# mkkellogg/GaussianSplats3D

Hardware: NVIDIA H100
Metric: frames_per_sec (higher is better)
Workload: dtype int32 sort keys / f32 raster

## Files before the change

gaussiansplats3d_b200/csrc/common.cuh:

```cuda
#pragma once
#include <cuda_runtime.h>
#include <stdint.h>
#include <stdio.h>
#include "../../include/gsplat_b200.h"

extern thread_local char g_gs_err[512];

#include <vector>
#include <string.h>
#include <stdlib.h>

namespace gs {

template <typename T, bool PINNED> struct GpuBuf {
    T *p = nullptr;
    size_t n = 0;
    GpuBuf() = default;
    GpuBuf(const GpuBuf &) = delete;
    GpuBuf &operator=(const GpuBuf &) = delete;
    ~GpuBuf() { release(); }
    int ensure(size_t count) {
        if (count <= n) return GS_OK;
        release();
        const size_t bytes = (count ? count : 1) * sizeof(T);
// ... 109 lines not shown
__device__ __forceinline__ uint32_t block_exclusive_scan(uint32_t v, uint32_t *smem_warp , uint32_t &total) {
    const int lane = threadIdx.x & 31, warp = threadIdx.x >> 5;
    constexpr int NW = THREADS / 32;
    const uint32_t inc = warp_inclusive_scan(v);
    if (lane == 31) smem_warp[warp] = inc;
    __syncthreads();
    if (warp == 0) {
        uint32_t w = lane < NW ? smem_warp[lane] : 0u;
        uint32_t wi = warp_inclusive_scan(w);
        smem_warp[lane] = wi - w;
        if (lane == 31) smem_warp[32] = wi;
    }
    __syncthreads();
    const uint32_t r = inc - v + smem_warp[warp];
    total = smem_warp[32];
    __syncthreads();
    return r;
}

struct SortControl {
    int32_t dmin, dmax;
    uint32_t error;
    uint32_t hist[4][kRadix];
};
constexpr uint32_t kErrDegenerate = 1u;
constexpr uint32_t kErrBucketRange = 2u;
constexpr uint32_t kErrCapacity = 4u;

}
```

gaussiansplats3d_b200/csrc/engine.cu:

```cuda
#include "../../include/gsplat_b200.h"
#include "common.cuh"
#include "sort_kernels.cuh"
#include "raster_kernels.cuh"
#include "shard_kernels.cuh"
#include "ksplat_transform.h"
#include "ksplat_kernels.cuh"
#include "file_kernels.cuh"
#include "cull_kernels.cuh"
#include "ray_kernels.cuh"
#include "generate_kernels.cuh"

#include <algorithm>
#include <cmath>
#include <cstdarg>
#include <cstdlib>
#include <cstring>
#include <memory>
#include <new>
#include <vector>

using namespace gs;

thread_local char g_gs_err[512] = "";
#define g_err g_gs_err
// ... 141 lines not shown
        if (graph_exec) cudaGraphExecDestroy(graph_exec);
        if (graph_exec_alt) cudaGraphExecDestroy(graph_exec_alt);
        for (cudaEvent_t x : ev) if (x) cudaEventDestroy(x);
        for (int i = 0; i < kPipeRing; ++i) { if (ev_frame_done[i]) cudaEventDestroy(ev_frame_done[i]); if (ev_copy_done[i]) cudaEventDestroy(ev_copy_done[i]); }
        for (cudaEvent_t x : {ev_params[0], ev_params[1], ev_fork, ev_join}) if (x) cudaEventDestroy(x);
        for (cudaStream_t x : {stream, stream2, copy_stream, param_stream}) if (x) cudaStreamDestroy(x);
    }
};

static int check_engine(gs_engine *e) {
    if (!e) return fail(GS_ERR_BAD_ARG, "null engine");
    cudaError_t ce = cudaSetDevice(e->cfg.device);
    if (ce != cudaSuccess) return fail(GS_ERR_CUDA, "cudaSetDevice(%d) -> %s", e->cfg.device, cudaGetErrorString(ce));
    return GS_OK;
}

extern "C" int gs_create(const gs_config *cfg, gs_engine **out) {
    if (!cfg || !out) return fail(GS_ERR_BAD_ARG, "gs_create: null argument");
    *out = nullptr;
    gs_config c{};
    memcpy(&c, cfg, std::min<size_t>(cfg->struct_size ? cfg->struct_size : sizeof(gs_config), sizeof(gs_config)));
    if (c.distance_map_range == 0) c.distance_map_range = 1u << 16;
    if (c.distance_map_range < 2 || c.distance_map_range > (1u << 24)) return fail(GS_ERR_BAD_ARG, "distance_map_range %u outside [2, 2^24]", c.distance_map_range);
    if (c.world_size == 0) { c.world_size = 1; c.rank = 0; }
    if (c.rank >= c.world_size) return fail(GS_ERR_BAD_ARG, "rank %u >= world_size %u", c.rank, c.world_size);
    int ndev = gs_device_count();
    if (ndev <= 0) return fail(GS_ERR_NO_DEVICE, "no CUDA device visible: libgsplat_b200 has no CPU path");
    if (c.device < 0 || c.device >= ndev) return fail(GS_ERR_BAD_ARG, "device %d not in [0,%d)", c.device, ndev);
    CU(cudaSetDevice(c.device));
    std::unique_ptr<gs_engine> e(new (std::nothrow) gs_engine());
    if (!e) return fail(GS_ERR_BAD_ARG, "out of host memory");
    e->cfg = c;
    cudaDeviceProp prop{};
    CU(cudaGetDeviceProperties(&prop, c.device));
    e->sm_count = prop.multiProcessorCount;
    if (prop.l2CacheSize > 0) e->l2_bytes = (size_t)prop.l2CacheSize;
    CU(cudaStreamCreateWithFlags(&e->stream, cudaStreamNonBlocking));
    CU(cudaStreamCreateWithFlags(&e->stream2, cudaStreamNonBlocking));
    CU(cudaEventCreateWithFlags(&e->ev_fork, cudaEventDisableTiming));
    CU(cudaEventCreateWithFlags(&e->ev_join, cudaEventDisableTiming));
    for (int i = 0; i < EV_COUNT; ++i) CU(cudaEventCreate(&e->ev[i]));
    int kb = 0;
    while ((1u << kb) < c.distance_map_range) ++kb;
    e->key_bits = kb;
    int rc = GS_OK;
    const size_t n = std::max<uint32_t>(c.max_splat_count, 1);
// ... 53 lines not shown
    P.irow[0] = (int32_t)((double)mvp[2] * 1000.0);
    P.irow[1] = (int32_t)((double)mvp[6] * 1000.0);
    P.irow[2] = (int32_t)((double)mvp[10] * 1000.0);
    P.irow[3] = 1;
    P.frow[0] = mvp[2]; P.frow[1] = mvp[6]; P.frow[2] = mvp[10]; P.frow[3] = 0.f;
    if (!capturing) CU(cudaMemcpyAsync(e->depthp.p + e->rs.frame_parity, &P, sizeof(P), cudaMemcpyHostToDevice, st));
    const bool integer = e->cfg.integer_based_sort, dyn = e->cfg.dynamic_mode;
    const int mode = use_pre ? (integer ? kIntPrecomputed : kFloatPrecomputed)
                             : (integer ? (dyn ? kIntDynamic : kIntStatic) : (dyn ? kFloatDynamic : kFloatStatic));
    const int dblocks = (int)std::max<uint64_t>(1, std::min<uint64_t>(((uint64_t)n + kDepthThreads * kDepthItems - 1) / (kDepthThreads * kDepthItems), (uint64_t)e->sm_count * 8));
    const bool identity = (d_indexes == nullptr);
    const void *pre = e->precomputed.p;
    switch (mode) {
        case kIntStatic: launch_depth<kIntStatic>(identity, dblocks, st, d_indexes, e->centers.p, pre, e->scene_idx.p, e->transforms.p, e->depthp.p + e->rs.frame_parity, lo, hi, e->dist.p, e->ctl.p); break;
        case kIntDynamic: launch_depth<kIntDynamic>(identity, dblocks, st, d_indexes, e->centers.p, pre, e->scene_idx.p, e->transforms.p, e->depthp.p + e->rs.frame_parity, lo, hi, e->dist.p, e->ctl.p); break;
        case kIntPrecomputed: launch_depth<kIntPrecomputed>(identity, dblocks, st, d_indexes, e->centers.p, pre, e->scene_idx.p, e->transforms.p, e->depthp.p + e->rs.frame_parity, lo, hi, e->dist.p, e->ctl.p); break;
        case kFloatStatic: launch_depth<kFloatStatic>(identity, dblocks, st, d_indexes, e->centers.p, pre, e->scene_idx.p, e->transforms.p, e->depthp.p + e->rs.frame_parity, lo, hi, e->dist.p, e->ctl.p); break;
        case kFloatDynamic: launch_depth<kFloatDynamic>(identity, dblocks, st, d_indexes, e->centers.p, pre, e->scene_idx.p, e->transforms.p, e->depthp.p + e->rs.frame_parity, lo, hi, e->dist.p, e->ctl.p); break;
        default: launch_depth<kFloatPrecomputed>(identity, dblocks, st, d_indexes, e->centers.p, pre, e->scene_idx.p, e->transforms.p, e->depthp.p + e->rs.frame_parity, lo, hi, e->dist.p, e->ctl.p); break;
    }
    return GS_OK;
}

static int sort_on_device(gs_engine *e, const uint32_t *d_indexes, const float *mvp, uint32_t sort_count, uint32_t render_count,
                          bool use_pre, bool write_buckets, bool capturing = false, bool subset = false, cudaEvent_t wait_for_rects = nullptr) {
    if (sort_count > render_count) return fail(GS_ERR_BAD_ARG, "sortCount %u > renderCount %u", sort_count, render_count);
    if (render_count > e->cfg.max_splat_count) return fail(GS_ERR_CAPACITY, "renderCount %u > max_splat_count %u", render_count, e->cfg.max_splat_count);
    cudaStream_t st = e->stream;
    const uint32_t s0 = render_count - sort_count, n = sort_count;
    const PassPlan pl = make_plan_bits(e->key_bits);
    uint32_t launches = 0;
    uint32_t stride = 0;
    int rc = e->tile_hist.ensure(radix_tile_hist_words(std::max(n, 1u), pl.npasses, &stride));
    if (rc) return rc;
    if (!capturing) CU(cudaEventRecord(e->ev[EV_SORT0], st));
    if (!e->have_prof_begin) e->prof.begin(st);
    if (e->ctl_dirty && !capturing) {
        gs_launch(k_sort_init, 1, 256, 0, st, e->ctl.p);
        ++launches;
    }
    if (!capturing) e->ctl_dirty = true;
    if (s0 > 0) { gs_launch(k_copy_head, std::min<uint32_t>((s0 + 255) / 256, e->sm_count * 8), 256, 0, st, d_indexes, e->sorted.p, s0); ++launches; e->prof.mark("k_copy_head", st); }
    if (n > 0) {
        if ((rc = enqueue_depth(e, d_indexes, mvp, use_pre, s0, render_count, capturing))) return rc;
        const bool identity = (d_indexes == nullptr);
        ++launches;
        e->prof.mark("k_depth", st);
        if (!capturing) CU(cudaEventRecord(e->ev[EV_DEPTH], st));
        const uint32_t tiles = (n + kRadixTile - 1) / kRadixTile;
        const uint32_t R = e->cfg.distance_map_range;
        const uint32_t *vsrc = identity ? nullptr : d_indexes + s0;
        int vmode = identity ? kValIotaReversed : kValArrayReversed;
        int32_t *dist_sorted = e->dist.p + s0;
        const unsigned long long *n_dev = nullptr;
        if (subset) {
            if (wait_for_rects) CU(cudaStreamWaitEvent(st, wait_for_rects, 0));
            int rcs = raster_subset(e->rs, e->cfg, d_indexes, render_count, e->dist.p, e->sub_idx.p, e->sub_dist.p, st, e->prof, launches);
            if (rcs) return rcs;
            vsrc = e->sub_idx.p; vmode = kValArrayReversed;
            dist_sorted = e->sub_dist.p;
            n_dev = &e->rs.rctl.p->subset_count;
        }
        static const RadixNames names = {{"k_radix_hist[depth,0]", "k_radix_hist[depth,1]", "k_radix_hist[depth,2]", "k_radix_hist[depth,3]"},
                                         {"k_radix_scan[depth,0]", "k_radix_scan[depth,1]", "k_radix_scan[depth,2]", "k_radix_scan[depth,3]"},
                                         {"k_radix_scatter[depth,0]", "k_radix_scatter[depth,1]", "k_radix_scatter[depth,2]", "k_radix_scatter[depth,3]"}};
        if (e->key_bits <= 16) {
            gs_launch(k_bucket<uint16_t>, tiles, kRadixThreads, 0, st, dist_sorted, (uint16_t *)e->keys[0].p, n, n_dev, R, pl, write_buckets ? 1 : 0, e->ctl.p, e->tile_hist.p, stride);
            ++launches;
            e->prof.mark("k_bucket", st);
            if (!capturing) CU(cudaEventRecord(e->ev[EV_BUCKET], st));
            radix_sort_pairs<uint16_t, uint32_t>((uint16_t *)e->keys[0].p, (uint16_t *)e->keys[1].p, vsrc, render_count - 1u, vmode, e->vals[0].p, e->vals[1].p,
                                       e->sorted.p + s0, n, n_dev, (unsigned long long)n, pl, e->ctl.p, e->tile_hist.p, stride, true, nullptr, st, launches, &e->prof, names, true);
        } else {
            gs_launch(k_bucket<uint32_t>, tiles, kRadixThreads, 0, st, dist_sorted, e->keys[0].p, n, n_dev, R, pl, write_buckets ? 1 : 0, e->ctl.p, e->tile_hist.p, stride);
            ++launches;
            e->prof.mark("k_bucket", st);
            if (!capturing) CU(cudaEventRecord(e->ev[EV_BUCKET], st));
            radix_sort_pairs<uint32_t, uint32_t>(e->keys[0].p, e->keys[1].p, vsrc, render_count - 1u, vmode, e->vals[0].p, e->vals[1].p, e->sorted.p + s0, n,
                                       n_dev, (unsigned long long)n, pl, e->ctl.p, e->tile_hist.p, stride, true, nullptr, st, launches, &e->prof, names, true);
        }
    } else if (!capturing) {
        CU(cudaEventRecord(e->ev[EV_DEPTH], st));
        CU(cudaEventRecord(e->ev[EV_BUCKET], st));
    }
    if (!capturing) CU(cudaEventRecord(e->ev[EV_SORT1], st));
    CU(cudaGetLastError());
    e->tm.kernel_launches = launches;
    e->last_render_count = render_count;
    e->have_sorted = true;
    if (!capturing) e->ctl_dirty = false;
    return GS_OK;
}

static int finish_sort(gs_engine *e, float *sort_time_ms) {
    CU(cudaMemcpyAsync(e->h_ctl.p, e->ctl.p, 12, cudaMemcpyDeviceToHost, e->stream));
    CU(cudaStreamSynchronize(e->stream));
    float ms = 0.f;
    if (e->last_frame_was_graph) {
        e->tm.depth_ms = e->tm.bucket_ms = e->tm.scatter_ms = 0.f;
        cudaEventElapsedTime(&ms, e->ev[EV_SORT0], e->ev[EV_R1]);
    } else {
        cudaEventElapsedTime(&e->tm.depth_ms, e->ev[EV_SORT0], e->ev[EV_DEPTH]);
        cudaEventElapsedTime(&e->tm.bucket_ms, e->ev[EV_DEPTH], e->ev[EV_BUCKET]);
// ... 47 lines not shown
    cudaEventElapsedTime(&e->tm.d2h_ms, e->ev[EV_D2H0], e->ev[EV_D2H1]);
    return rc;
}


static int shard_prepare(gs_engine *e) {
    const uint32_t R = e->cfg.distance_map_range;
    int rc;
    const size_t bytes = sizeof(ShardHeader) + (size_t)R * sizeof(uint2);
    if (e->shard.block.n < bytes) {
        if ((rc = e->shard.block.ensure(bytes))) return rc;
        CU(cudaMemset(e->shard.block.p, 0, bytes));
    }
    const size_t blocks = ((size_t)R + kShardScanThreads - 1) / kShardScanThreads;
    if ((rc = e->shard.total.ensure(R)) || (rc = e->shard.ahead.ensure(R)) || (rc = e->shard.delta.ensure(R)) || (rc = e->shard.block_total.ensure(blocks)) ||
        (rc = e->shard.local_sorted.ensure(e->cfg.max_splat_count)))
        return rc;
    const PassPlan pl = make_plan_bits(e->key_bits);
    if ((rc = e->tile_hist.ensure(radix_tile_hist_words(std::max(e->cfg.max_splat_count, 1u), pl.npasses, nullptr))) || (rc = e->precomputed.ensure(e->cfg.max_splat_count))) return rc;
    return GS_OK;
}
template <typename F> static inline void preload_kernel(F f) { cudaFuncAttributes a; (void)cudaFuncGetAttributes(&a, f); }
template <typename KeyT> static void shard_preload_keyed() {
    preload_kernel(k_bucket<KeyT>);
    preload_kernel(k_radix_hist<KeyT>);
    preload_kernel(k_shard_place<KeyT>);
    preload_kernel(k_radix_scatter<KeyT, uint32_t, kValArray, true, false>);
    preload_kernel(k_radix_scatter<KeyT, uint32_t, kValArrayReversed, true, false>);
    preload_kernel(k_radix_scatter<KeyT, uint32_t, kValIotaReversed, true, false>);
    preload_kernel(k_radix_scatter<KeyT, uint32_t, kValArray, true, true>);
    preload_kernel(k_radix_scatter<KeyT, uint32_t, kValArrayReversed, true, true>);
    preload_kernel(k_radix_scatter<KeyT, uint32_t, kValIotaReversed, true, true>);
}
template <int MODE> static void shard_preload_depth() { preload_kernel(k_depth<MODE, true>); preload_kernel(k_depth<MODE, false>); }
static void shard_preload(gs_engine *e) {
    preload_kernel(k_sort_init); preload_kernel(k_copy_head); preload_kernel(k_radix_scan);
    preload_kernel(k_shard_exchange_minmax); preload_kernel(k_shard_exchange_runs); preload_kernel(k_shard_totals); preload_kernel(k_shard_delta); preload_kernel(k_shard_done);
    shard_preload_depth<kIntStatic>(); shard_preload_depth<kIntDynamic>(); shard_preload_depth<kIntPrecomputed>();
    shard_preload_depth<kFloatStatic>(); shard_preload_depth<kFloatDynamic>(); shard_preload_depth<kFloatPrecomputed>();
    if (e->key_bits <= 16) shard_preload_keyed<uint16_t>(); else shard_preload_keyed<uint32_t>();
    (void)cudaGetLastError();
}
static inline ShardHeader *shard_hdr(void *block) { return (ShardHeader *)block; }
static inline const uint2 *shard_runs(void *block) { return (const uint2 *)((unsigned char *)block + sizeof(ShardHeader)); }

extern "C" int gs_shard_export(gs_engine *e, void *block_handle, void *sorted_handle) {
    int rc = check_engine(e);
// ... 62 lines not shown
        if ((rc = shard_prepare(pe))) return rc;
        blocks[g] = pe->shard.block.p;
    }
    return shard_bind(e, world, blocks, engines[0]->sorted.p);
}

template <typename KeyT>
static int shard_local_sort(gs_engine *e, const uint32_t *d_indexes, uint32_t s0, uint32_t lo, uint32_t hi, uint32_t &launches) {
    cudaStream_t st = e->stream;
    const uint32_t n = hi - lo, R = e->cfg.distance_map_range;
    const PassPlan pl = make_plan_bits(e->key_bits);
    uint32_t stride = 0;
    int rc = e->tile_hist.ensure(radix_tile_hist_words(std::max(n, 1u), pl.npasses, &stride));
    if (rc) return rc;
    const bool identity = (d_indexes == nullptr);
    static const RadixNames names = {{"k_radix_hist[shard,0]", "k_radix_hist[shard,1]", "k_radix_hist[shard,2]", "k_radix_hist[shard,3]"},
                                     {"k_radix_scan[shard,0]", "k_radix_scan[shard,1]", "k_radix_scan[shard,2]", "k_radix_scan[shard,3]"},
                                     {"k_radix_scatter[shard,0]", "k_radix_scatter[shard,1]", "k_radix_scatter[shard,2]", "k_radix_scatter[shard,3]"}};
    const uint32_t me = e->cfg.rank, world = e->shard.world, seq = e->shard.seq;
    uint2 *runs = (uint2 *)shard_runs(e->shard.block.p);
    KeyT *final_keys = nullptr;
    if (n) {
        const uint32_t tiles = (n + kRadixTile - 1) / kRadixTile;
        gs_launch(k_bucket<KeyT>, tiles, kRadixThreads, 0, st, e->dist.p + lo, (KeyT *)e->keys[0].p, n, nullptr, R, pl, 0, e->ctl.p, e->tile_hist.p, stride);
        ++launches;
        e->prof.mark("k_bucket", st);
        radix_sort_pairs<KeyT, uint32_t>((KeyT *)e->keys[0].p, (KeyT *)e->keys[1].p, identity ? nullptr : d_indexes + lo, hi - 1u,
                                         identity ? kValIotaReversed : kValArrayReversed, e->vals[0].p, e->vals[1].p, e->shard.local_sorted.p, n, nullptr,
                                         (unsigned long long)n, pl, e->ctl.p, e->tile_hist.p, stride, true, runs, st, launches, &e->prof, names, true, true, &final_keys);
    }
    k_shard_exchange_runs<<<1, 32, 0, st>>>(e->shard.peers, me, world, seq);
    ++launches;
    e->prof.mark("k_shard_exchange_runs", st);
    if (n) {
        const uint32_t sblocks = (R + kShardScanThreads - 1) / kShardScanThreads;
        k_shard_totals<<<sblocks, kShardScanThreads, 0, st>>>(e->shard.peers, me, world, R, e->shard.total.p, e->shard.ahead.p, e->shard.block_total.p);
        k_shard_delta<<<sblocks, kShardScanThreads, 0, st>>>(runs, R, e->shard.total.p, e->shard.ahead.p, e->shard.block_total.p, e->shard.delta.p);
        e->prof.mark("k_shard_offsets", st);
        k_shard_place<KeyT><<<std::min<uint32_t>((n + 255) / 256, e->sm_count * 16), 256, 0, st>>>(final_keys, e->shard.local_sorted.p, n, e->shard.delta.p, e->shard.root_out + s0);
        e->prof.mark("k_shard_place", st);
        launches += 3;
    }
    return GS_OK;
}

static inline uint32_t shard_bound(uint32_t s0, uint32_t n, uint32_t g, uint32_t world) { return s0 + (uint32_t)(((uint64_t)n * g) / world); }

// ... 1465 lines not shown
```

gaussiansplats3d_b200/csrc/sort_kernels.cuh:

```cuda
#pragma once
#include "common.cuh"

namespace gs {

enum DepthMode : int {
    kIntStatic = 0, kIntDynamic = 1, kIntPrecomputed = 2, kFloatStatic = 3, kFloatDynamic = 4, kFloatPrecomputed = 5
};

struct DepthParams {
    int32_t irow[4];
    float frow[4];
    float mvp[16];
};

__global__ void k_sort_init(SortControl *ctl) {
    pdl_enter();
    const uint32_t tid = threadIdx.x;
    if (tid == 0) {
        ctl->dmin = 2147483640;
        ctl->dmax = -2147483640;
        ctl->error = 0;
    }
    uint32_t *h = &ctl->hist[0][0];
    for (uint32_t i = tid; i < 4 * kRadix; i += blockDim.x) h[i] = 0;
// ... 51 lines not shown
    DepthParams P;
#pragma unroll
    for (int i = 0; i < 4; ++i) { P.irow[i] = __ldg(&Pp->irow[i]); P.frow[i] = __ldg(&Pp->frow[i]); }
    if (MODE == kIntDynamic || MODE == kFloatDynamic) {
#pragma unroll
        for (int i = 0; i < 16; ++i) P.mvp[i] = __ldg(&Pp->mvp[i]);
    }
    __shared__ int32_t s_irow[GS_MAX_SCENES_DEV][4];
    __shared__ float s_frow[GS_MAX_SCENES_DEV][4];
    __shared__ int s_min[kDepthThreads / 32], s_max[kDepthThreads / 32];
    if (MODE == kIntDynamic || MODE == kFloatDynamic) {
        if (threadIdx.x < GS_MAX_SCENES_DEV) {
            float row[4];
            scene_row(P.mvp, transforms + 16 * threadIdx.x, row);
#pragma unroll
            for (int k = 0; k < 4; ++k) {
                s_frow[threadIdx.x][k] = row[k];
                s_irow[threadIdx.x][k] = trunc_scaled(row[k], 1000.0);
            }
        }
        __syncthreads();
    }
    if (blockIdx.x == 0 && threadIdx.x == 0) ctl->error = 0;
    int32_t lmin = 2147483640, lmax = -2147483640;
    const uint32_t tile = kDepthThreads * kDepthItems;
    for (uint64_t base = (uint64_t)s0 + (uint64_t)blockIdx.x * tile; base < rc; base += (uint64_t)gridDim.x * tile) {
        uint32_t g[kDepthItems];
#pragma unroll
        for (int k = 0; k < kDepthItems; ++k) {
            const uint64_t i = base + (uint64_t)k * kDepthThreads + threadIdx.x;
            g[k] = (i < rc) ? (IDENTITY ? (uint32_t)i : ld_nc_u32(indexes + i)) : 0xffffffffu;
        }
        int32_t d[kDepthItems];
#pragma unroll
        for (int k = 0; k < kDepthItems; ++k)
            if (g[k] != 0xffffffffu) d[k] = splat_distance<MODE>(g[k], centers, pre, scene_idx, P, s_irow, s_frow);
#pragma unroll
        for (int k = 0; k < kDepthItems; ++k) {
            const uint64_t i = base + (uint64_t)k * kDepthThreads + threadIdx.x;
            if (i < rc) {
                dist[i] = d[k];
                lmin = min(lmin, d[k]);
                lmax = max(lmax, d[k]);
            }
        }
    }
// ... 6 lines not shown
        lmax = threadIdx.x < kDepthThreads / 32 ? s_max[threadIdx.x] : -2147483640;
        lmin = warp_min(lmin);
        lmax = warp_max(lmax);
        if (threadIdx.x == 0) {
            atomicMin(&ctl->dmin, lmin);
            atomicMax(&ctl->dmax, lmax);
        }
    }
}

struct PassPlan {
    int npasses;
    int shift[4];
    int bits[4];
};

constexpr int kRadixThreads = 512;
constexpr int kRadixItems = 8;
constexpr int kRadixTile = kRadixThreads * kRadixItems;
constexpr int kRadixWarps = kRadixThreads / 32;

enum ValMode : int { kValArray = 0, kValArrayReversed = 1, kValIotaReversed = 2 };

template <int NB>
__device__ __forceinline__ uint32_t warp_peers(uint32_t d) {
    uint32_t peers = 0xffffffffu;
#pragma unroll
    for (int b = 0; b < NB; ++b) {
        const bool bit = (d >> b) & 1u;
        const uint32_t vote = __ballot_sync(0xffffffffu, bit);
        peers &= bit ? vote : ~vote;
    }
    return peers;
}

template <typename KeyT>
__global__ void __launch_bounds__(kRadixThreads)
k_bucket(int32_t *__restrict__ dist , KeyT *__restrict__ keys, uint32_t n_host,
         const unsigned long long *__restrict__ n_dev, uint32_t R, PassPlan plan, int write_buckets, SortControl *ctl,
         uint32_t *__restrict__ tile_hist, uint32_t stride) {
    pdl_enter();
    __shared__ uint32_t s_hist[kRadix];
    if (threadIdx.x < kRadix) s_hist[threadIdx.x] = 0;
    __syncthreads();
    const int32_t dmin = ctl->dmin, dmax = ctl->dmax;
    const float span = __fsub_rn(__int2float_rn(dmax), __int2float_rn(dmin));
    const float range_map = __fdiv_rn(__uint2float_rn(R - 1u), span);
    const bool degenerate = (dmax == dmin);
    uint32_t err = 0;
    const uint32_t n = n_dev ? (uint32_t)*n_dev : n_host;
    const uint64_t jbase = (uint64_t)blockIdx.x * kRadixTile;
    int32_t d[kRadixItems];
#pragma unroll
    for (int k = 0; k < kRadixItems; ++k) {
        const uint64_t j = jbase + (uint64_t)k * kRadixThreads + threadIdx.x;
        d[k] = (j < n) ? dist[(uint64_t)n - 1u - j] : 0;
    }
#pragma unroll
    for (int k = 0; k < kRadixItems; ++k) {
        const uint64_t j = jbase + (uint64_t)k * kRadixThreads + threadIdx.x;
        if (j < n) {
            const int32_t rel = (int32_t)((uint32_t)d[k] - (uint32_t)dmin);
            int32_t b = __float2int_rz(__fmul_rn(__int2float_rn(rel), range_map));
            if (degenerate) b = 0;
            if (rel < 0 || b < 0) { err |= kErrBucketRange; b = 0; }
            else if ((uint32_t)b >= R) b = (int32_t)(R - 1u);
            if (write_buckets) dist[(uint64_t)n - 1u - j] = b;
            const uint32_t key = (R - 1u) - (uint32_t)b;
            keys[j] = (KeyT)key;
            atomicAdd(&s_hist[(key >> plan.shift[0]) & ((1u << plan.bits[0]) - 1u)], 1u);
        }
    }
    __syncthreads();
    if (threadIdx.x < kRadix) {
        const uint32_t v = s_hist[threadIdx.x];
        tile_hist[(size_t)threadIdx.x * stride + blockIdx.x] = v;
        if (v) atomicAdd(&ctl->hist[0][threadIdx.x], v);
    }
    if (err) atomicOr(&ctl->error, err);
    if (degenerate && blockIdx.x == 0 && threadIdx.x == 0) atomicOr(&ctl->error, kErrDegenerate);
}

template <typename KeyT>
__global__ void __launch_bounds__(kRadixThreads)
k_radix_hist(const KeyT *__restrict__ keys, uint32_t n_host, const unsigned long long *__restrict__ n_dev, unsigned long long n_cap,
             int shift, int bits, uint32_t *__restrict__ tile_hist, uint32_t stride, uint32_t *global_hist, int add_global) {
    pdl_enter();
    const uint32_t n = n_dev ? (uint32_t)min(*n_dev, n_cap) : n_host;
    const uint64_t base = (uint64_t)blockIdx.x * kRadixTile;
    if (base >= n) return;
    __shared__ uint32_t s_hist[kRadix];
    if (threadIdx.x < kRadix) s_hist[threadIdx.x] = 0;
    __syncthreads();
    const uint32_t dmask = (1u << bits) - 1u;
    uint32_t kk[kRadixItems];
#pragma unroll
    for (int k = 0; k < kRadixItems; ++k) {
        const uint64_t e = base + (uint64_t)k * kRadixThreads + threadIdx.x;
// ... 21 lines not shown
    const uint32_t ntiles = (uint32_t)(((uint64_t)n + kRadixTile - 1) / kRadixTile);
    const uint32_t d = blockIdx.x;
    {
        uint32_t total;
        const uint32_t c = (threadIdx.x < kRadix && threadIdx.x < d) ? global_hist[threadIdx.x] : 0u;
        (void)block_exclusive_scan<kScanColThreads>(c, s_scan, total);
        if (threadIdx.x == 0) s_carry = total;
    }
    __syncthreads();
    uint32_t *col = tile_hist + (size_t)d * stride;
    for (uint32_t base = 0; base < ntiles; base += kScanColThreads) {
        const uint32_t t = base + threadIdx.x;
        const uint32_t v = t < ntiles ? col[t] : 0u;
        uint32_t total;
        const uint32_t ex = block_exclusive_scan<kScanColThreads>(v, s_scan, total);
        const uint32_t carry = s_carry;
        if (t < ntiles) col[t] = ex + carry;
        __syncthreads();
        if (threadIdx.x == 0) s_carry = carry + total;
        __syncthreads();
    }
}

template <typename KeyT, typename ValT, int VALMODE, bool WRITE_KEYS, bool RANGES, bool FULL>
__device__ __forceinline__ void radix_scatter_tile(const KeyT *__restrict__ keys_in, const ValT *__restrict__ vals_in, uint32_t iota_top,
                                                   KeyT *__restrict__ keys_out, ValT *__restrict__ vals_out, uint32_t n, uint32_t tile,
                                                   int shift, uint32_t dmask, const uint32_t *__restrict__ tile_offsets, uint32_t stride,
                                                   uint2 *ranges, unsigned char *s_raw, uint32_t *s_tile_count, uint32_t *s_tile_start,
                                                   uint32_t *s_gbase, uint32_t *s_scan) {
    uint32_t(*s_whist)[kRadix + 1] = reinterpret_cast<uint32_t(*)[kRadix + 1]>(s_raw);
    ValT *s_vals = reinterpret_cast<ValT *>(s_raw);
    KeyT *s_keys = reinterpret_cast<KeyT *>(s_raw + (size_t)kRadixTile * sizeof(ValT));
    const int tid = threadIdx.x, lane = tid & 31, warp = tid >> 5;
    const uint32_t tile_base = tile * (uint32_t)kRadixTile;
    const uint32_t run_base = tile_base + (uint32_t)warp * (32 * kRadixItems) + lane;
    for (int i = tid; i < kRadixWarps * (kRadix + 1); i += kRadixThreads) (&s_whist[0][0])[i] = 0;

    uint32_t key[kRadixItems];
#pragma unroll
    for (int k = 0; k < kRadixItems; ++k) {
        const uint32_t e = run_base + (uint32_t)k * 32;
        key[k] = (FULL || e < n) ? (uint32_t)keys_in[e] : 0xffffffffu;
    }
    const uint32_t my_offset = tid < kRadix ? tile_offsets[(size_t)tid * stride + tile] : 0u;
    uint32_t peers[kRadixItems];
#pragma unroll
    for (int k = 0; k < kRadixItems; ++k) {
        const uint32_t d = (FULL || key[k] != 0xffffffffu) ? ((key[k] >> shift) & dmask) : (uint32_t)kRadix;
        peers[k] = warp_peers<FULL ? 8 : 9>(d);
    }
    __syncthreads();
    uint32_t rank[kRadixItems];
    const uint32_t lt = lanemask_lt();
#pragma unroll
    for (int k = 0; k < kRadixItems; ++k) {
        const uint32_t d = (FULL || key[k] != 0xffffffffu) ? ((key[k] >> shift) & dmask) : (uint32_t)kRadix;
        const uint32_t before = s_whist[warp][d];
        rank[k] = before + __popc(peers[k] & lt);
        __syncwarp();
        if ((peers[k] & lt) == 0) s_whist[warp][d] = before + __popc(peers[k]);
        __syncwarp();
    }
    __syncthreads();
    if (tid < kRadix) {
        uint32_t run = 0;
#pragma unroll
        for (int w = 0; w < kRadixWarps; ++w) {
            const uint32_t c = s_whist[w][tid];
            s_whist[w][tid] = run;
            run += c;
        }
        s_tile_count[tid] = run;
    }
    __syncthreads();
    {
        uint32_t total;
        const uint32_t c = tid < kRadix ? s_tile_count[tid] : 0u;
        const uint32_t ex = block_exclusive_scan<kRadixThreads>(c, s_scan, total);
        if (tid < kRadix) { s_tile_start[tid] = ex; s_gbase[tid] = my_offset - ex; }
    }
    __syncthreads();
#pragma unroll
    for (int k = 0; k < kRadixItems; ++k) {
        const uint32_t d = (key[k] >> shift) & dmask;
        rank[k] = (FULL || key[k] != 0xffffffffu) ? (s_tile_start[d] + s_whist[warp][d] + rank[k]) : 0xffffffffu;
    }
    __syncthreads();
#pragma unroll
    for (int k = 0; k < kRadixItems; ++k) {
        const uint32_t e = run_base + (uint32_t)k * 32;
        if (FULL || rank[k] != 0xffffffffu) {
            ValT v;
            if (VALMODE == kValArray) v = __ldg(vals_in + e);
            else if (VALMODE == kValArrayReversed) v = __ldg(vals_in + (n - 1u - e));
            else v = (ValT)(iota_top - e);
            s_vals[rank[k]] = v;
            s_keys[rank[k]] = (KeyT)key[k];
        }
    }
    __syncthreads();
    const uint32_t valid = FULL ? (uint32_t)kRadixTile : (n - tile_base);
#pragma unroll
    for (int k = 0; k < kRadixItems; ++k) {
        const uint32_t q = (uint32_t)k * kRadixThreads + tid;
// ... 20 lines not shown
    pdl_enter();
    const uint32_t n = n_dev ? (uint32_t)min(*n_dev, n_cap) : n_host;
    const uint32_t tile = blockIdx.x;
    if (tile == 0) {
        if (clear_hist && threadIdx.x < kRadix) clear_hist[threadIdx.x] = 0;
        if (reset_ctl && threadIdx.x == 0) { reset_ctl->dmin = 2147483640; reset_ctl->dmax = -2147483640; }
    }
    const uint64_t tile_base = (uint64_t)tile * kRadixTile;
    if (tile_base >= n) return;
    __shared__ __align__(16) unsigned char s_raw[kRadixTile * (sizeof(KeyT) + sizeof(ValT)) > kRadixWarps * (kRadix + 1) * 4
                                                     ? kRadixTile * (sizeof(KeyT) + sizeof(ValT))
                                                     : kRadixWarps * (kRadix + 1) * 4];
    __shared__ uint32_t s_tile_count[kRadix];
    __shared__ uint32_t s_tile_start[kRadix];
    __shared__ uint32_t s_gbase[kRadix];
    __shared__ uint32_t s_scan[40];
    const uint32_t dmask = (1u << bits) - 1u;
    if (tile_base + kRadixTile <= n)
        radix_scatter_tile<KeyT, ValT, VALMODE, WRITE_KEYS, RANGES, true>(keys_in, vals_in, iota_top, keys_out, vals_out, n, tile, shift, dmask, tile_offsets, stride,
                                                                          ranges, s_raw, s_tile_count, s_tile_start, s_gbase, s_scan);
    else
        radix_scatter_tile<KeyT, ValT, VALMODE, WRITE_KEYS, RANGES, false>(keys_in, vals_in, iota_top, keys_out, vals_out, n, tile, shift, dmask, tile_offsets, stride,
                                                                           ranges, s_raw, s_tile_count, s_tile_start, s_gbase, s_scan);
}

__global__ void k_copy_head(const uint32_t *__restrict__ indexes, uint32_t *__restrict__ out, uint32_t s0) {
    pdl_enter();
    for (uint64_t i = (uint64_t)blockIdx.x * blockDim.x + threadIdx.x; i < s0; i += (uint64_t)gridDim.x * blockDim.x)
        out[i] = indexes ? indexes[i] : (uint32_t)i;
}

__global__ void k_bucket_counts(const int32_t *__restrict__ buckets, uint32_t s0, uint32_t rc, uint32_t *counts) {
    for (uint64_t i = (uint64_t)s0 + (uint64_t)blockIdx.x * blockDim.x + threadIdx.x; i < rc; i += (uint64_t)gridDim.x * blockDim.x)
        atomicAdd(&counts[buckets[i]], 1u);
}
__global__ void __launch_bounds__(1024) k_exclusive_scan_single_block(uint32_t *data, uint32_t n) {
    __shared__ uint32_t s_scan[40];
    __shared__ uint32_t s_carry;
    if (threadIdx.x == 0) s_carry = 0;
    __syncthreads();
    for (uint32_t base = 0; base < n; base += 1024) {
        const uint32_t i = base + threadIdx.x;
        const uint32_t v = i < n ? data[i] : 0u;
        uint32_t total;
        const uint32_t ex = block_exclusive_scan<1024>(v, s_scan, total);
        const uint32_t carry = s_carry;
// ... 79 lines not shown
    ValT *vt[2] = {vtmp0, vtmp1};
    for (int p = 0; p < pl.npasses; ++p) {
        const bool last = (p == pl.npasses - 1);
        ValT *vout = last ? vals_final : vt[p & 1];
        uint32_t *th = tile_hist + (size_t)p * kRadix * stride;
        if (!(p == 0 && hist0_done)) {
            gs_launch(k_radix_hist<KeyT>, tiles, kRadixThreads, 0, st, kin, n, n_dev, n_cap, pl.shift[p], pl.bits[p], th, stride, &ctl->hist[p][0], 1);
            ++launches;
            if (prof) prof->mark(names.hist[p], st);
        }
        gs_launch(k_radix_scan, 1u << pl.bits[p], kScanColThreads, 0, st, th, stride, n, n_dev, n_cap, &ctl->hist[p][0]);
        ++launches;
        if (prof) prof->mark(names.scan[p], st);
        if (last && final_keys) *final_keys = kout;
        launch_radix_scatter<KeyT, ValT>(tiles, p == 0, !last || keep_final_keys, last && ranges != nullptr, first_valmode, kin, vin, iota_top, kout, vout, n, n_dev, n_cap,
                                   pl.shift[p], pl.bits[p], th, stride, ranges, self_clean ? &ctl->hist[p][0] : nullptr,
                                   (self_clean && last) ? ctl : nullptr, st);
        ++launches;
        if (prof) prof->mark(names.scatter[p], st);
        vin = vout;
        KeyT *t = kin; kin = kout; kout = t;
    }
}
static inline size_t radix_tile_hist_words(unsigned long long n, int npasses, uint32_t *stride_out) {
    const size_t tiles = (size_t)((n + kRadixTile - 1) / kRadixTile);
    const size_t stride = (tiles + 31) & ~(size_t)31;
    if (stride_out) *stride_out = (uint32_t)stride;
    return stride * kRadix * (size_t)npasses;
}

}
```

Before: 3257.

## Replace per-pass hist/scan/scatter depth sort with onesweep decoupled look-back radix sort

For sorts up to 4M keys, the bucket kernel now builds histograms for every digit pass at once. Each pass then runs a single onesweep kernel that takes tile indices dynamically and computes global digit offsets through decoupled look-back over per-tile status words. This drops the separate histogram and scan launches for each pass, which cuts launch count and global traffic. The cost is spin-waiting in the look-back and a new 30-bit count limit on max_splat_count, now checked at engine creation.

```diff
diff --git a/gaussiansplats3d_b200/csrc/common.cuh b/gaussiansplats3d_b200/csrc/common.cuh
--- a/gaussiansplats3d_b200/csrc/common.cuh
+++ b/gaussiansplats3d_b200/csrc/common.cuh
@@ -155,6 +155,7 @@
     int32_t dmin, dmax;
     uint32_t error;
     uint32_t hist[4][kRadix];
+    uint32_t tile_seq[4];
 };
 constexpr uint32_t kErrDegenerate = 1u;
 constexpr uint32_t kErrBucketRange = 2u;
diff --git a/gaussiansplats3d_b200/csrc/engine.cu b/gaussiansplats3d_b200/csrc/engine.cu
--- a/gaussiansplats3d_b200/csrc/engine.cu
+++ b/gaussiansplats3d_b200/csrc/engine.cu
@@ -187,6 +187,7 @@
     memcpy(&c, cfg, std::min<size_t>(cfg->struct_size ? cfg->struct_size : sizeof(gs_config), sizeof(gs_config)));
     if (c.distance_map_range == 0) c.distance_map_range = 1u << 16;
     if (c.distance_map_range < 2 || c.distance_map_range > (1u << 24)) return fail(GS_ERR_BAD_ARG, "distance_map_range %u outside [2, 2^24]", c.distance_map_range);
+    if (c.max_splat_count > kLbCount) return fail(GS_ERR_BAD_ARG, "max_splat_count %u above 2^30 - 1 (the depth sort's 30-bit digit counts)", c.max_splat_count);
     if (c.world_size == 0) { c.world_size = 1; c.rank = 0; }
     if (c.rank >= c.world_size) return fail(GS_ERR_BAD_ARG, "rank %u >= world_size %u", c.rank, c.world_size);
     int ndev = gs_device_count();
@@ -286,6 +287,32 @@
     return GS_OK;
 }
 
+constexpr uint32_t kOneSweepMaxKeys = 4u << 20;
+
+template <typename KeyT>
+static int enqueue_bucket_radix(gs_engine *e, int32_t *dist_sorted, const uint32_t *vsrc, int vmode, uint32_t iota_top, uint32_t *out, uint32_t n,
+                                const unsigned long long *n_dev, const PassPlan &pl, uint32_t stride, bool write_buckets, bool capturing, uint32_t &launches) {
+    static const RadixNames names = {{"k_radix_hist[depth,0]", "k_radix_hist[depth,1]", "k_radix_hist[depth,2]", "k_radix_hist[depth,3]"},
+                                     {"k_radix_scan[depth,0]", "k_radix_scan[depth,1]", "k_radix_scan[depth,2]", "k_radix_scan[depth,3]"},
+                                     {"k_radix_scatter[depth,0]", "k_radix_scatter[depth,1]", "k_radix_scatter[depth,2]", "k_radix_scatter[depth,3]"}};
+    cudaStream_t st = e->stream;
+    const uint32_t tiles = (n + kRadixTile - 1) / kRadixTile;
+    KeyT *k0 = (KeyT *)e->keys[0].p, *k1 = (KeyT *)e->keys[1].p;
+    const bool onesweep = n <= kOneSweepMaxKeys;
+    gs_launch(onesweep ? k_bucket<KeyT, true> : k_bucket<KeyT, false>, tiles, kRadixThreads, 0, st, dist_sorted, k0, n, n_dev, e->cfg.distance_map_range, pl,
+              write_buckets ? 1 : 0, e->ctl.p, e->tile_hist.p, stride);
+    ++launches;
+    e->prof.mark("k_bucket", st);
+    if (!capturing) CU(cudaEventRecord(e->ev[EV_BUCKET], st));
+    if (onesweep)
+        radix_sort_onesweep<KeyT>(k0, k1, vsrc, iota_top, vmode, e->vals[0].p, e->vals[1].p, out, n, n_dev, pl, e->ctl.p, e->tile_hist.p, stride, st, launches,
+                                  &e->prof, names.scatter);
+    else
+        radix_sort_pairs<KeyT, uint32_t>(k0, k1, vsrc, iota_top, vmode, e->vals[0].p, e->vals[1].p, out, n, n_dev, (unsigned long long)n, pl, e->ctl.p, e->tile_hist.p,
+                                         stride, true, nullptr, st, launches, &e->prof, names, true);
+    return GS_OK;
+}
+
 static int sort_on_device(gs_engine *e, const uint32_t *d_indexes, const float *mvp, uint32_t sort_count, uint32_t render_count,
                           bool use_pre, bool write_buckets, bool capturing = false, bool subset = false, cudaEvent_t wait_for_rects = nullptr) {
     if (sort_count > render_count) return fail(GS_ERR_BAD_ARG, "sortCount %u > renderCount %u", sort_count, render_count);
@@ -311,8 +338,6 @@
         ++launches;
         e->prof.mark("k_depth", st);
         if (!capturing) CU(cudaEventRecord(e->ev[EV_DEPTH], st));
-        const uint32_t tiles = (n + kRadixTile - 1) / kRadixTile;
-        const uint32_t R = e->cfg.distance_map_range;
         const uint32_t *vsrc = identity ? nullptr : d_indexes + s0;
         int vmode = identity ? kValIotaReversed : kValArrayReversed;
         int32_t *dist_sorted = e->dist.p + s0;
@@ -325,24 +350,9 @@
             dist_sorted = e->sub_dist.p;
             n_dev = &e->rs.rctl.p->subset_count;
         }
-        static const RadixNames names = {{"k_radix_hist[depth,0]", "k_radix_hist[depth,1]", "k_radix_hist[depth,2]", "k_radix_hist[depth,3]"},
-                                         {"k_radix_scan[depth,0]", "k_radix_scan[depth,1]", "k_radix_scan[depth,2]", "k_radix_scan[depth,3]"},
-                                         {"k_radix_scatter[depth,0]", "k_radix_scatter[depth,1]", "k_radix_scatter[depth,2]", "k_radix_scatter[depth,3]"}};
-        if (e->key_bits <= 16) {
-            gs_launch(k_bucket<uint16_t>, tiles, kRadixThreads, 0, st, dist_sorted, (uint16_t *)e->keys[0].p, n, n_dev, R, pl, write_buckets ? 1 : 0, e->ctl.p, e->tile_hist.p, stride);
-            ++launches;
-            e->prof.mark("k_bucket", st);
-            if (!capturing) CU(cudaEventRecord(e->ev[EV_BUCKET], st));
-            radix_sort_pairs<uint16_t, uint32_t>((uint16_t *)e->keys[0].p, (uint16_t *)e->keys[1].p, vsrc, render_count - 1u, vmode, e->vals[0].p, e->vals[1].p,
-                                       e->sorted.p + s0, n, n_dev, (unsigned long long)n, pl, e->ctl.p, e->tile_hist.p, stride, true, nullptr, st, launches, &e->prof, names, true);
-        } else {
-            gs_launch(k_bucket<uint32_t>, tiles, kRadixThreads, 0, st, dist_sorted, e->keys[0].p, n, n_dev, R, pl, write_buckets ? 1 : 0, e->ctl.p, e->tile_hist.p, stride);
-            ++launches;
-            e->prof.mark("k_bucket", st);
-            if (!capturing) CU(cudaEventRecord(e->ev[EV_BUCKET], st));
-            radix_sort_pairs<uint32_t, uint32_t>(e->keys[0].p, e->keys[1].p, vsrc, render_count - 1u, vmode, e->vals[0].p, e->vals[1].p, e->sorted.p + s0, n,
-                                       n_dev, (unsigned long long)n, pl, e->ctl.p, e->tile_hist.p, stride, true, nullptr, st, launches, &e->prof, names, true);
-        }
+        rc = (e->key_bits <= 16) ? enqueue_bucket_radix<uint16_t>(e, dist_sorted, vsrc, vmode, render_count - 1u, e->sorted.p + s0, n, n_dev, pl, stride, write_buckets, capturing, launches)
+                                 : enqueue_bucket_radix<uint32_t>(e, dist_sorted, vsrc, vmode, render_count - 1u, e->sorted.p + s0, n, n_dev, pl, stride, write_buckets, capturing, launches);
+        if (rc) return rc;
     } else if (!capturing) {
         CU(cudaEventRecord(e->ev[EV_DEPTH], st));
         CU(cudaEventRecord(e->ev[EV_BUCKET], st));
@@ -436,7 +446,7 @@
 }
 template <typename F> static inline void preload_kernel(F f) { cudaFuncAttributes a; (void)cudaFuncGetAttributes(&a, f); }
 template <typename KeyT> static void shard_preload_keyed() {
-    preload_kernel(k_bucket<KeyT>);
+    preload_kernel(k_bucket<KeyT, false>);
     preload_kernel(k_radix_hist<KeyT>);
     preload_kernel(k_shard_place<KeyT>);
     preload_kernel(k_radix_scatter<KeyT, uint32_t, kValArray, true, false>);
@@ -545,7 +555,7 @@
     KeyT *final_keys = nullptr;
     if (n) {
         const uint32_t tiles = (n + kRadixTile - 1) / kRadixTile;
-        gs_launch(k_bucket<KeyT>, tiles, kRadixThreads, 0, st, e->dist.p + lo, (KeyT *)e->keys[0].p, n, nullptr, R, pl, 0, e->ctl.p, e->tile_hist.p, stride);
+        gs_launch(k_bucket<KeyT, false>, tiles, kRadixThreads, 0, st, e->dist.p + lo, (KeyT *)e->keys[0].p, n, nullptr, R, pl, 0, e->ctl.p, e->tile_hist.p, stride);
         ++launches;
         e->prof.mark("k_bucket", st);
         radix_sort_pairs<KeyT, uint32_t>((KeyT *)e->keys[0].p, (KeyT *)e->keys[1].p, identity ? nullptr : d_indexes + lo, hi - 1u,
diff --git a/gaussiansplats3d_b200/csrc/sort_kernels.cuh b/gaussiansplats3d_b200/csrc/sort_kernels.cuh
--- a/gaussiansplats3d_b200/csrc/sort_kernels.cuh
+++ b/gaussiansplats3d_b200/csrc/sort_kernels.cuh
@@ -97,6 +97,8 @@
         __syncthreads();
     }
     if (blockIdx.x == 0 && threadIdx.x == 0) ctl->error = 0;
+    if (blockIdx.x == 0)
+        for (uint32_t i = threadIdx.x; i < 4 * kRadix; i += kDepthThreads) (&ctl->hist[0][0])[i] = 0;
     int32_t lmin = 2147483640, lmax = -2147483640;
     const uint32_t tile = kDepthThreads * kDepthItems;
     for (uint64_t base = (uint64_t)s0 + (uint64_t)blockIdx.x * tile; base < rc; base += (uint64_t)gridDim.x * tile) {
@@ -149,6 +151,11 @@
 
 enum ValMode : int { kValArray = 0, kValArrayReversed = 1, kValIotaReversed = 2 };
 
+constexpr uint32_t kLbAggregate = 1u << 30;
+constexpr uint32_t kLbInclusive = 2u << 30;
+constexpr uint32_t kLbCount = (1u << 30) - 1u;
+constexpr int kLookbackWindow = 16;
+
 template <int NB>
 __device__ __forceinline__ uint32_t warp_peers(uint32_t d) {
     uint32_t peers = 0xffffffffu;
@@ -161,14 +168,19 @@
     return peers;
 }
 
-template <typename KeyT>
+template <typename KeyT, bool ONESWEEP>
 __global__ void __launch_bounds__(kRadixThreads)
 k_bucket(int32_t *__restrict__ dist , KeyT *__restrict__ keys, uint32_t n_host,
          const unsigned long long *__restrict__ n_dev, uint32_t R, PassPlan plan, int write_buckets, SortControl *ctl,
          uint32_t *__restrict__ tile_hist, uint32_t stride) {
     pdl_enter();
-    __shared__ uint32_t s_hist[kRadix];
-    if (threadIdx.x < kRadix) s_hist[threadIdx.x] = 0;
+    __shared__ uint32_t s_hist[ONESWEEP ? 3 : 1][kRadix];
+    if (ONESWEEP) {
+        for (int i = threadIdx.x; i < 3 * kRadix; i += kRadixThreads) (&s_hist[0][0])[i] = 0;
+        if (threadIdx.x < kRadix)
+            for (int p = 0; p < plan.npasses; ++p) tile_hist[((size_t)p * stride + blockIdx.x) * kRadix + threadIdx.x] = 0;
+        if (blockIdx.x == 0 && threadIdx.x < 4) ctl->tile_seq[threadIdx.x] = 0;
+    } else if (threadIdx.x < kRadix) s_hist[0][threadIdx.x] = 0;
     __syncthreads();
     const int32_t dmin = ctl->dmin, dmax = ctl->dmax;
     const float span = __fsub_rn(__int2float_rn(dmax), __int2float_rn(dmin));
@@ -195,12 +207,22 @@
             if (write_buckets) dist[(uint64_t)n - 1u - j] = b;
             const uint32_t key = (R - 1u) - (uint32_t)b;
             keys[j] = (KeyT)key;
-            atomicAdd(&s_hist[(key >> plan.shift[0]) & ((1u << plan.bits[0]) - 1u)], 1u);
-        }
-    }
-    __syncthreads();
-    if (threadIdx.x < kRadix) {
-        const uint32_t v = s_hist[threadIdx.x];
+            if (ONESWEEP) {
+#pragma unroll
+                for (int p = 0; p < 3; ++p)
+                    if (p < plan.npasses) atomicAdd(&s_hist[p][(key >> plan.shift[p]) & ((1u << plan.bits[p]) - 1u)], 1u);
+            } else
+                atomicAdd(&s_hist[0][(key >> plan.shift[0]) & ((1u << plan.bits[0]) - 1u)], 1u);
+        }
+    }
+    __syncthreads();
+    if (ONESWEEP) {
+        for (int i = threadIdx.x; i < plan.npasses * kRadix; i += kRadixThreads) {
+            const uint32_t v = (&s_hist[0][0])[i];
+            if (v) atomicAdd(&ctl->hist[0][0] + i, v);
+        }
+    } else if (threadIdx.x < kRadix) {
+        const uint32_t v = s_hist[0][threadIdx.x];
         tile_hist[(size_t)threadIdx.x * stride + blockIdx.x] = v;
         if (v) atomicAdd(&ctl->hist[0][threadIdx.x], v);
     }
@@ -268,12 +290,39 @@
     }
 }
 
-template <typename KeyT, typename ValT, int VALMODE, bool WRITE_KEYS, bool RANGES, bool FULL>
+__device__ __forceinline__ uint32_t ld_relaxed_gpu_u32(const uint32_t *p) {
+    uint32_t r;
+    asm volatile("ld.relaxed.gpu.global.u32 %0, [%1];" : "=r"(r) : "l"(p) : "memory");
+    return r;
+}
+__device__ __forceinline__ void st_relaxed_gpu_u32(uint32_t *p, uint32_t v) {
+    asm volatile("st.relaxed.gpu.global.u32 [%0], %1;" ::"l"(p), "r"(v) : "memory");
+}
+
+__device__ __forceinline__ uint32_t lookback_exclusive(const uint32_t *digit_status , uint32_t tile) {
+    uint32_t sum = 0;
+    int j = (int)tile - 1;
+    for (;;) {
+        uint32_t v[kLookbackWindow];
+#pragma unroll
+        for (int i = 0; i < kLookbackWindow; ++i) v[i] = (j - i >= 0) ? ld_relaxed_gpu_u32(digit_status + (size_t)(j - i) * kRadix) : kLbInclusive;
+#pragma unroll
+        for (int i = 0; i < kLookbackWindow; ++i) {
+            const uint32_t flag = v[i] & ~kLbCount;
+            if (flag == 0) break;
+            sum += v[i] & kLbCount;
+            --j;
+            if (flag == kLbInclusive) return sum;
+        }
+    }
+}
+
+template <typename KeyT, typename ValT, int VALMODE, bool WRITE_KEYS, bool RANGES, bool FULL, bool ONESWEEP = false>
 __device__ __forceinline__ void radix_scatter_tile(const KeyT *__restrict__ keys_in, const ValT *__restrict__ vals_in, uint32_t iota_top,
                                                    KeyT *__restrict__ keys_out, ValT *__restrict__ vals_out, uint32_t n, uint32_t tile,
                                                    int shift, uint32_t dmask, const uint32_t *__restrict__ tile_offsets, uint32_t stride,
                                                    uint2 *ranges, unsigned char *s_raw, uint32_t *s_tile_count, uint32_t *s_tile_start,
-                                                   uint32_t *s_gbase, uint32_t *s_scan) {
+                                                   uint32_t *s_gbase, uint32_t *s_scan, uint32_t *lb_status = nullptr, uint32_t digit_total = 0) {
     uint32_t(*s_whist)[kRadix + 1] = reinterpret_cast<uint32_t(*)[kRadix + 1]>(s_raw);
     ValT *s_vals = reinterpret_cast<ValT *>(s_raw);
     KeyT *s_keys = reinterpret_cast<KeyT *>(s_raw + (size_t)kRadixTile * sizeof(ValT));
@@ -288,7 +337,7 @@
         const uint32_t e = run_base + (uint32_t)k * 32;
         key[k] = (FULL || e < n) ? (uint32_t)keys_in[e] : 0xffffffffu;
     }
-    const uint32_t my_offset = tid < kRadix ? tile_offsets[(size_t)tid * stride + tile] : 0u;
+    const uint32_t my_offset = (!ONESWEEP && tid < kRadix) ? tile_offsets[(size_t)tid * stride + tile] : 0u;
     uint32_t peers[kRadixItems];
 #pragma unroll
     for (int k = 0; k < kRadixItems; ++k) {
@@ -317,15 +366,29 @@
             run += c;
         }
         s_tile_count[tid] = run;
+        if (ONESWEEP) st_relaxed_gpu_u32(lb_status + (size_t)tile * kRadix + tid, (tile == 0 ? kLbInclusive : kLbAggregate) | run);
     }
     __syncthreads();
     {
         uint32_t total;
-        const uint32_t c = tid < kRadix ? s_tile_count[tid] : 0u;
+        const uint32_t c = tid < kRadix ? s_tile_count[tid] : (ONESWEEP ? digit_total : 0u);
         const uint32_t ex = block_exclusive_scan<kRadixThreads>(c, s_scan, total);
-        if (tid < kRadix) { s_tile_start[tid] = ex; s_gbase[tid] = my_offset - ex; }
-    }
-    __syncthreads();
+        if (ONESWEEP) {
+            static_assert(kRadixThreads == 2 * kRadix, "one look-back thread per digit in the upper half of the CTA");
+            if (tid < kRadix) s_tile_start[tid] = ex;
+            else {
+                const uint32_t d = (uint32_t)tid - kRadix;
+                uint32_t before = 0;
+                if (tile) {
+                    before = lookback_exclusive(lb_status + d, tile);
+                    st_relaxed_gpu_u32(lb_status + (size_t)tile * kRadix + d, kLbInclusive | (before + s_tile_count[d]));
+                }
+                s_gbase[d] = ex - (FULL ? (uint32_t)kRadixTile : n - tile_base) + before;
+            }
+        } else if (tid < kRadix) { s_tile_start[tid] = ex; s_gbase[tid] = my_offset - ex; }
+    }
+    __syncthreads();
+    if (ONESWEEP && tid < kRadix) s_gbase[tid] -= s_tile_start[tid];
 #pragma unroll
     for (int k = 0; k < kRadixItems; ++k) {
         const uint32_t d = (key[k] >> shift) & dmask;
@@ -392,6 +455,39 @@
     else
         radix_scatter_tile<KeyT, ValT, VALMODE, WRITE_KEYS, RANGES, false>(keys_in, vals_in, iota_top, keys_out, vals_out, n, tile, shift, dmask, tile_offsets, stride,
                                                                            ranges, s_raw, s_tile_count, s_tile_start, s_gbase, s_scan);
+}
+
+template <typename KeyT, typename ValT, int VALMODE, bool WRITE_KEYS>
+__global__ void __launch_bounds__(kRadixThreads, 2)
+k_radix_onesweep(const KeyT *__restrict__ keys_in, const ValT *__restrict__ vals_in, uint32_t iota_top, KeyT *__restrict__ keys_out,
+                 ValT *__restrict__ vals_out, uint32_t n_host, const unsigned long long *__restrict__ n_dev, int pass, int shift, int bits,
+                 uint32_t *lb_status , SortControl *ctl, int reseed) {
+    pdl_enter();
+    __shared__ __align__(16) unsigned char s_raw[kRadixTile * (sizeof(KeyT) + sizeof(ValT)) > kRadixWarps * (kRadix + 1) * 4
+                                                     ? kRadixTile * (sizeof(KeyT) + sizeof(ValT))
+                                                     : kRadixWarps * (kRadix + 1) * 4];
+    __shared__ uint32_t s_tile_count[kRadix];
+    __shared__ uint32_t s_tile_start[kRadix];
+    __shared__ uint32_t s_gbase[kRadix];
+    __shared__ uint32_t s_scan[40];
+    __shared__ uint32_t s_tile;
+    if (threadIdx.x == 0) {
+        s_tile = atomicAdd(&ctl->tile_seq[pass], 1u);
+        if (reseed && blockIdx.x == 0) { ctl->dmin = 2147483640; ctl->dmax = -2147483640; }
+    }
+    const uint32_t digit_total = threadIdx.x >= kRadix ? ctl->hist[pass][threadIdx.x - kRadix] : 0u;
+    const uint32_t n = n_dev ? (uint32_t)min(*n_dev, (unsigned long long)n_host) : n_host;
+    __syncthreads();
+    const uint32_t tile = s_tile;
+    const uint64_t tile_base = (uint64_t)tile * kRadixTile;
+    if (tile_base >= n) return;
+    const uint32_t dmask = (1u << bits) - 1u;
+    if (tile_base + kRadixTile <= n)
+        radix_scatter_tile<KeyT, ValT, VALMODE, WRITE_KEYS, false, true, true>(keys_in, vals_in, iota_top, keys_out, vals_out, n, tile, shift, dmask, nullptr, 0,
+                                                                               nullptr, s_raw, s_tile_count, s_tile_start, s_gbase, s_scan, lb_status, digit_total);
+    else
+        radix_scatter_tile<KeyT, ValT, VALMODE, WRITE_KEYS, false, false, true>(keys_in, vals_in, iota_top, keys_out, vals_out, n, tile, shift, dmask, nullptr, 0,
+                                                                                nullptr, s_raw, s_tile_count, s_tile_start, s_gbase, s_scan, lb_status, digit_total);
 }
 
 __global__ void k_copy_head(const uint32_t *__restrict__ indexes, uint32_t *__restrict__ out, uint32_t s0) {
@@ -517,6 +613,35 @@
         KeyT *t = kin; kin = kout; kout = t;
     }
 }
+
+template <typename KeyT>
+static void radix_sort_onesweep(KeyT *keys0, KeyT *keys1, const uint32_t *vals_src, uint32_t iota_top, int first_valmode, uint32_t *vtmp0,
+                                uint32_t *vtmp1, uint32_t *vals_final, uint32_t n, const unsigned long long *n_dev, const PassPlan &pl,
+                                SortControl *ctl, uint32_t *tile_hist, uint32_t stride, cudaStream_t st, uint32_t &launches, Profiler *prof,
+                                const char *const *names) {
+    const uint32_t tiles = (uint32_t)(((uint64_t)n + kRadixTile - 1) / kRadixTile);
+    if (!tiles) return;
+    KeyT *kin = keys0, *kout = keys1;
+    const uint32_t *vin = vals_src;
+    uint32_t *vt[2] = {vtmp0, vtmp1};
+    for (int p = 0; p < pl.npasses; ++p) {
+        const bool last = (p == pl.npasses - 1);
+        uint32_t *vout = last ? vals_final : vt[p & 1];
+        uint32_t *status = tile_hist + (size_t)p * stride * kRadix;
+        const int vm = p == 0 ? first_valmode : kValArray;
+#define GS_PASS(VM, WK) gs_launch(k_radix_onesweep<KeyT, uint32_t, VM, WK>, tiles, kRadixThreads, 0, st, kin, vin, iota_top, kout, vout, n, n_dev, p, \
+                                  pl.shift[p], pl.bits[p], status, ctl, last ? 1 : 0)
+        if (vm == kValArray) { if (last) GS_PASS(kValArray, false); else GS_PASS(kValArray, true); }
+        else if (vm == kValArrayReversed) { if (last) GS_PASS(kValArrayReversed, false); else GS_PASS(kValArrayReversed, true); }
+        else { if (last) GS_PASS(kValIotaReversed, false); else GS_PASS(kValIotaReversed, true); }
+#undef GS_PASS
+        ++launches;
+        if (prof) prof->mark(names[p], st);
+        vin = vout;
+        KeyT *t = kin; kin = kout; kout = t;
+    }
+}
+
 static inline size_t radix_tile_hist_words(unsigned long long n, int npasses, uint32_t *stride_out) {
     const size_t tiles = (size_t)((n + kRadixTile - 1) / kRadixTile);
     const size_t stride = (tiles + 31) & ~(size_t)31;
```

Measured after the change: 3336 (median of 6 runs). +2.4%, better.
